# jdm365/Compression_Algorithms

Hardware: AMD Instinct MI355X
Metric: encode GB/s on enwik9 at 1/2/4/8 MI355X; ratio vs ref; round-trip bit-exact (higher is better)
Workload: dtype u8; 1 GPU; deflate (LZ77 W=32 KiB len<=31 + per-block dynamic Huffman over the 286-symbol alphabet, mode H), independent 64 KiB blocks; 1000000000 enwik-shaped bytes in the job, 1000000000 on rank 0; input_seed=12345, mode=H, input_bytes_job=1000000000, input_bytes_rank0=1000000000, compressed_bytes_job=516875560, compressed_bytes_rank0=516875560, gather_to_rank0=False, parallelism=blocks sharded over 1 GPU(s), weak scaling

## Files before the change

compression_algorithms_amd/csrc/lz2.h:

```cpp
#pragma once
#include "lz_common.h"

#define LZ2_NG_BITS   14
#define LZ2_NG        (1u << LZ2_NG_BITS)
#ifndef LZ2_CAP
#define LZ2_CAP       4096u
#endif
#ifndef LZ2_CAP_S
#define LZ2_CAP_S     2048u
#endif
#ifndef LZ2_THREADS
#define LZ2_THREADS   512
#endif
#define LZ2_NWAVES    (LZ2_THREADS / 64)
#ifndef LZ2_PARTBITS
#define LZ2_PARTBITS  7
#endif
#define LZ2_MAXPARTS  (1u << LZ2_PARTBITS)
static_assert(LZ2_CAP % LZ2_THREADS == 0 && LZ2_CAP_S % LZ2_THREADS == 0 && LZ2_CAP_S <= LZ2_CAP, "entries per thread must be whole");
static_assert(2u * (LZ_MAX_BLOCK / LZ2_CAP_S + 1u + 16u) + 2u <= LZ2_MAXPARTS, "a block could need more parts than the partition can number");
#define LZ2_GRID_PARTS 40u
static_assert(LZ2_GRID_PARTS * LZ2_CAP_S >= 5u * LZ_MAX_BLOCK / 4u, "the grid must cover a full block of text with room to spare");
#ifndef LZ2_BIG
#define LZ2_BIG       8u
#endif
#define LZ2_WAVE      128u
#define LZ2_MAXBIG    (LZ2_CAP / LZ2_BIG)
#define LZ2_BIG_STRIDE (2u * LZ_MAX_BLOCK)
#define LZ2_ALIGN8(x)  (((x) + 7u) & ~7u)
#define LZ2_DESC_SMALL (LZ_MAX_BLOCK / LZ2_BIG + 32u)
#define LZ2_NCLASS    8u
#define LZ2_BIG_SMALL 1024u
__host__ __device__ __forceinline__ uint32_t lz2_class_of(uint32_t cnt, uint32_t wave_min)
{
    const bool three = (wave_min >> 16) != 0u;
    wave_min &= 0xFFFFu;
    if (cnt >= wave_min) return cnt > LZ2_BIG_SMALL ? 6u : cnt >= 512u ? 4u : (three && cnt < 256u) ? 3u : 5u;
    return cnt < 16 ? 7u : cnt < 32 ? 0u : cnt < 64 ? 1u : cnt < 128 ? 2u : cnt < 256 ? 3u : 4u;
}

struct Lz2BlockMeta {
    uint32_t n, nparts, base, fallback;
    uint32_t nbig, nbig_entries;
    uint32_t pad[2];
    uint32_t part_start[LZ2_MAXPARTS];
    uint32_t part_count[LZ2_MAXPARTS];
    uint32_t part_lo[LZ2_MAXPARTS];
};

struct Lz2BigDesc {
    uint32_t block;
    uint32_t start;
    uint32_t count;
    uint32_t anom;
    uint32_t limit;
    uint32_t pad[3];
};

struct Lz2Scratch {
    uint8_t      *partmap;
    uint16_t     *plist;
    uint16_t     *cand;
    Lz2BlockMeta *meta;
    uint32_t     *fallback_count, *fallback_list;
    uint32_t     *work_count;
    uint32_t      work_slots;
    uint64_t     *work;
    uint16_t     *bigpos, *bigrs, *bigpid, *bigcand;
    Lz2BigDesc   *desc[LZ2_NCLASS];
    uint32_t     *big_count;
    uint64_t     *dbg;
    uint32_t      wave_min;
    uint32_t      stop_phase;
};
```

compression_algorithms_amd/csrc/lz2_find.hip:

```cpp
#include "lz_common.h"
#include "lz2.h"
#include "lz_dom.h"
#include "lz_replay.h"
#include <stdlib.h>

#define RS_HEAD 0x8000u
#define RS_MASK 0x7FFFu

__device__ __forceinline__ bool bm2_test(const uint32_t *bm, uint32_t b) { return (bm[b >> 5] >> (b & 31u)) & 1u; }

__device__ void replay_small(const uint16_t *pos, uint16_t *rs, const uint16_t *pid, uint16_t *occ, uint32_t *bm,
                             uint32_t s, uint32_t e, uint32_t W, uint32_t anom, uint32_t limit, uint16_t *cand_i)
{
    uint32_t ev = s;
    bool anom_pending = anom != ~0u;
    const bool plain = (anom == ~0u) && (limit == ~0u);
    if (plain && (uint32_t)pos[e - 1] <= (uint32_t)pos[s] + W) {
        for (uint32_t i = s; i < e; ++i) { const uint32_t id = pid[i]; cand_i[i] = (id != pos[i]) ? (uint16_t)id : (uint16_t)LZ_NONE16; }
        return;
    }
    for (uint32_t i = s; i < e; ++i) {
        const uint32_t p = pos[i], rsv = rs[i], r = rsv & RS_MASK, id = pid[i];
        while (ev < i && (uint32_t)pos[ev] + W < p) {
            const uint32_t b = rs[ev] & RS_MASK;
// ... 581 lines not shown
        lz2_find_part<LZ2_CAP>(in, n_total, P, sc, block0, k < nwide ? sc.work[sc.work_slots - 1u - k] : sc.work[covered + (k - nwide)]);
        __syncthreads();
    }
}

template <int LDS_ENTRIES, int NW>
__global__ __launch_bounds__(64)
void k_lz2_big(LzP P, Lz2Scratch sc, int large)
{
    __shared__ uint32_t s_occ[LDS_ENTRIES];
    __shared__ uint16_t s_slot[LDS_ENTRIES];
    const uint32_t lane = threadIdx.x;
    const uint32_t nhi = large == 1 ? sc.big_count[6] : (large == 2 || large == 4) ? 0u : sc.big_count[4],
                   ncl = nhi + ((large == 0 || large == 2) ? sc.big_count[5] : large == 4 ? sc.big_count[3] : 0u);
    const uint32_t W = 1u << P.wbits;
    for (uint32_t ci = blockIdx.x; ci < ncl; ci += gridDim.x) {
        const Lz2BigDesc *dp = large == 1 ? &sc.desc[6][ci] : large == 4 ? &sc.desc[3][ci] : (ci < nhi ? &sc.desc[4][ci] : &sc.desc[5][ci - nhi]);
        const uint32_t d_block = dp->block, d_start = dp->start, n = dp->count;
        if (n & 0x80000000u) continue;
        const uint32_t d_anom = dp->anom, d_limit = dp->limit;
        const uint16_t *bp = sc.bigpos + (size_t)d_block * LZ2_BIG_STRIDE + d_start;
        const uint16_t *br = sc.bigrs + (size_t)d_block * LZ2_BIG_STRIDE + d_start;
        const uint16_t *bi = sc.bigpid + (size_t)d_block * LZ2_BIG_STRIDE + d_start;
        uint16_t *bc = sc.bigcand + (size_t)d_block * LZ2_BIG_STRIDE + d_start;
        const bool plain = d_anom == ~0u && d_limit == ~0u;
        if constexpr (NW > 1) {
            if (n <= 2048u) {
                if (plain) big_replay<LDS_ENTRIES, 1, true>(s_occ, s_slot, lane, W, n, d_anom, d_limit, bp, br, bi, bc);
                else big_replay<LDS_ENTRIES, 1, false>(s_occ, s_slot, lane, W, n, d_anom, d_limit, bp, br, bi, bc);
                continue;
            }
            if (n <= 4096u) {
                if (plain) big_replay<LDS_ENTRIES, 2, true>(s_occ, s_slot, lane, W, n, d_anom, d_limit, bp, br, bi, bc);
                else big_replay<LDS_ENTRIES, 2, false>(s_occ, s_slot, lane, W, n, d_anom, d_limit, bp, br, bi, bc);
                continue;
            }
        }
        if (plain) big_replay<LDS_ENTRIES, NW, true>(s_occ, s_slot, lane, W, n, d_anom, d_limit, bp, br, bi, bc);
        else big_replay<LDS_ENTRIES, NW, false>(s_occ, s_slot, lane, W, n, d_anom, d_limit, bp, br, bi, bc);
    }
}

#define LZ2_DOM_DONE 0x80000000u
__global__ __launch_bounds__(256)
void k_lz2_dom(LzP P, Lz2Scratch sc)
{
    constexpr uint32_t RING = LZ2_CAP;
    static_assert((RING & (RING - 1u)) == 0, "the ring is indexed with a mask");
    __shared__ uint32_t s_occ[LZ2_CAP / 32 + 72 + 264];
    __shared__ uint16_t s_ring[RING];
    __shared__ uint16_t s_fid[DOM_FCAP], s_fpos[DOM_FCAP], s_fslot[DOM_FCAP];
    __shared__ uint32_t s_votes[3], s_result, s_next;
    const uint32_t tid = threadIdx.x;
    const uint32_t W = 1u << P.wbits;
    const uint32_t count = sc.big_count[6];
    uint32_t *cursor = sc.big_count + 8;
    struct Src {
        const uint16_t *bp, *br, *bi; uint16_t *bc;
        __device__ __forceinline__ uint64_t ent(uint32_t i) const { return ((uint64_t)bp[i] << 16) | ((uint64_t)br[i] << 32) | ((uint64_t)bi[i] << 48); }
        __device__ __forceinline__ void put(uint32_t i, uint32_t, uint32_t res) const { bc[i] = (uint16_t)res; }
    };
    for (;;) {
        __syncthreads();
        if (tid == 0) s_next = atomicAdd(cursor, 1u);
        __syncthreads();
        const uint32_t ci = s_next;
        if (ci >= count) break;
        Lz2BigDesc *dp = &sc.desc[6][ci];
        const uint32_t m = dp->count;
        if (dp->anom != ~0u || dp->limit != ~0u || m > LZ2_CAP) continue;
        const size_t at = (size_t)dp->block * LZ2_BIG_STRIDE + dp->start;
        Src src{sc.bigpos + at, sc.bigrs + at, sc.bigpid + at, sc.bigcand + at};
        for (uint32_t i = tid; i < m; i += 256) src.bc[i] = (uint16_t)LZ_NONE16;
        if (tid == 0) { s_votes[0] = s_votes[1] = s_votes[2] = 0; s_result = 0; }
        __syncthreads();
        const bool done = dom_cluster(src, m, W, (W < RING ? W : RING) - 1u, s_occ, s_ring, s_fid, s_fpos, s_fslot, s_votes, s_result, nullptr);
        if (done && tid == 0) dp->count = m | LZ2_DOM_DONE;
    }
}

#define ROW_BPERM(src_lane, v) ((uint32_t)__builtin_amdgcn_ds_bpermute((int)((src_lane) << 2), (int)(v)))

template <int RL>
__device__ __forceinline__ uint32_t row_first_zero(uint32_t v, uint32_t from, uint32_t l, uint32_t rb)
{
    constexpr uint32_t RMASK = RL == 32 ? 0xFFFFFFFFu : ((1u << (RL & 31)) - 1u);
    const uint32_t rw = from >> 5, lowmask = (1u << (from & 31u)) - 1u;
    if (l < rw) v = 0xFFFFFFFFu; else if (l == rw) v |= lowmask;
    const uint64_t mk = __ballot(v != 0xFFFFFFFFu);
    const uint32_t my = (uint32_t)(mk >> rb) & RMASK;
    const uint32_t ln = my ? (uint32_t)__builtin_ctz(my) : 0u;
    const uint32_t mv = ROW_BPERM(rb + ln, v);
    const uint32_t fz = (mv != 0xFFFFFFFFu) ? (uint32_t)__builtin_ctz(~mv) : 0u;
    return my ? ((ln << 5) + fz) : ~0u;
}

template <int RL>
__global__ __launch_bounds__(64)
void k_lz2_rows(LzP P, Lz2Scratch sc, int cls_a, int cls_b, int cursor_slot)
{
    static_assert(RL == 8 || RL == 16 || RL == 32, "rows of 8, 16 or 32 lanes");
    constexpr int NR = 64 / RL, CAPE = 32 * RL;
    constexpr uint32_t RMASK = RL == 32 ? 0xFFFFFFFFu : ((1u << (RL & 31)) - 1u);
    __shared__ uint32_t s_occ[NR][CAPE];
    __shared__ uint32_t s_ent[NR][CAPE];
    __shared__ uint32_t s_bm[NR][RL];
    const uint32_t lane = threadIdx.x, g = lane / (uint32_t)RL, l = lane & (uint32_t)(RL - 1), rb = lane & ~(uint32_t)(RL - 1);
    const uint32_t W = 1u << P.wbits;
    const uint32_t count_a = sc.big_count[cls_a], count = count_a + sc.big_count[cls_b];
    uint32_t *cursor = sc.big_count + cursor_slot;
    Lz2BigDesc *const descs_a = sc.desc[cls_a], *const descs_b = sc.desc[cls_b];
    auto desc_of = [&](uint32_t ticket) -> Lz2BigDesc * { return ticket < count_a ? descs_a + ticket : descs_b + (ticket - count_a); };
    uint32_t *occ = s_occ[g], *ent = s_ent[g], *bmw = s_bm[g];

    bool active = false, exhausted = false;
    uint32_t n = 0, i0 = 0, ev = 0;
    size_t at = 0;
    uint32_t cur_a = 0, cur_b = 0, out_acc = LZ_NONE16;
    uint32_t pf_stage = 0, pf_ci = 0, pf_count = 0;
    size_t pf_at = 0;
    uint32_t r_np = 0, r_ni = 0, r_nr = 0, r_fp = 0, r_fi = 0, r_fr = 0, tk = 0;
    uint4 r_d4 = make_uint4(0, 0, 0, 0); uint32_t r_d1 = 0;
    uint32_t vzero;
    asm volatile("v_mov_b32 %0, 0" : "=v"(vzero));

    for (;;) {
        const bool flush = active && i0 + l < n;
        uint16_t *const flush_to = sc.bigcand + at + i0 + l;
        if (active) {
            i0 += (uint32_t)RL;
            if (i0 >= n) active = false;
            else { cur_a = r_np | (r_ni << 16); cur_b = r_nr; }
        }
        bool take = false, want_cursor = false;
        uint32_t done_ci = 0, done_n = 0;
        if (!active && pf_stage == 3u) {
            take = true;
            n = pf_count; at = pf_at;
            cur_a = r_fp | (r_fi << 16); cur_b = r_fr; i0 = 0; ev = 0; active = true; pf_stage = 0;
            bmw[l] = 0;
            done_ci = pf_ci; done_n = n;
        }
        if (pf_stage == 1u) {
            pf_ci = ROW_BPERM(rb, tk);
            if (pf_ci >= count) { exhausted = true; pf_stage = 0; } else pf_stage = 2;
        } else if (pf_stage == 2u) {
            if (r_d4.w != ~0u || r_d1 != ~0u || r_d4.z > (uint32_t)CAPE || r_d4.z < 2u * RL) pf_stage = 0;
            else { pf_count = r_d4.z; pf_at = (size_t)r_d4.x * LZ2_BIG_STRIDE + r_d4.y; pf_stage = 3; }
        }
        if (pf_stage == 0u && !exhausted) { want_cursor = true; pf_stage = 1; }
        {
            const uint32_t k = i0 + (uint32_t)RL + l;
            const size_t na = (active && k < n) ? at + k : 0;
            r_np = sc.bigpos[na]; r_ni = sc.bigpid[na]; r_nr = sc.bigrs[na];
            const size_t fa = (pf_stage == 3u) ? pf_at + l : 0;
            r_fp = sc.bigpos[fa]; r_fi = sc.bigpid[fa]; r_fr = sc.bigrs[fa];
            const uint32_t *dp = reinterpret_cast<const uint32_t *>(pf_stage == 2u ? desc_of(pf_ci) : descs_a);
            r_d4 = *reinterpret_cast<const uint4 *>(dp); r_d1 = dp[4];
        }
        if (flush) *flush_to = (uint16_t)out_acc;
        if (take && l == 0) desc_of(done_ci)->count = done_n | LZ2_DOM_DONE;
        if (want_cursor && l == 0) tk = atomicAdd(cursor + vzero, 1u);
        if (__ballot(active || pf_stage != 0u) == 0ull) break;
        if (__ballot(active) == 0ull) continue;
        uint32_t a = ROW_BPERM(rb, cur_a), r = ROW_BPERM(rb, cur_b);
        uint32_t e = ent[(active && ev + l < i0) ? ev + l : 0u];
        for (uint32_t t = 0; t < (uint32_t)RL; ++t) {
            const uint32_t i = i0 + t;
            const bool on = active && i < n;
            const uint32_t p = a & 0xFFFFu, id = a >> 16;
            for (;;) {
                const bool ret = on && ev + l < i && (e >> 16) + W < p;
                const uint64_t mk = __ballot(ret);
                if (ret) atomicAnd(&bmw[(e & 0xFFFFu) >> 5], ~(1u << (e & 31u)));
                const uint32_t cnt = (uint32_t)__popc((uint32_t)(mk >> rb) & RMASK);
                ev += cnt;
                if (__ballot(cnt == (uint32_t)RL) == 0ull) break;
                e = ent[(on && ev + l < i) ? ev + l : 0u];
            }
            const uint32_t wr = bmw[r >> 5], h = occ[r], v = bmw[l];
            const uint32_t tn = (t + 1u) & (uint32_t)(RL - 1);
            const uint32_t na = ROW_BPERM(rb + tn, cur_a), nr = ROW_BPERM(rb + tn, cur_b);
            const bool bit = (wr >> (r & 31u)) & 1u, same = (h & 0xFFFFu) == id;
            const bool seek = on && id != p;
            uint32_t res = (seek && ev == 0u) ? id : (seek && bit && same) ? (h >> 16) : (uint32_t)LZ_NONE16;
            bool walk = seek && ev != 0u && bit && !same;
            if (__ballot(walk) != 0ull) {
                uint32_t e_end = row_first_zero<RL>(v, r + 1u, l, rb);
                if (e_end > (uint32_t)CAPE) e_end = (uint32_t)CAPE;
                uint32_t b0 = r + 1u;
                while (__ballot(walk && b0 < e_end) != 0ull) {
                    const uint32_t bb = b0 + l;
                    const bool in = walk && bb < e_end;
                    const uint32_t o = occ[in ? bb : 0u];
                    const uint64_t mk = __ballot(in && (o & 0xFFFFu) == id);
                    const uint32_t my = (uint32_t)(mk >> rb) & RMASK;
                    const uint32_t src = ROW_BPERM(rb + (my ? (uint32_t)__builtin_ctz(my) : 0u), o);
                    if (walk && my) { res = src >> 16; walk = false; }
                    b0 += (uint32_t)RL;
                }
            }
            const uint32_t b = row_first_zero<RL>(v, r, l, rb);
            const bool put = on && b < (uint32_t)CAPE;
            if (put && l == 0) atomicOr(&bmw[b >> 5], 1u << (b & 31u));
            if (put) { occ[b] = id | (p << 16); ent[i] = b | (p << 16); }
            if (on && l == t) out_acc = res;
            e = ent[(active && i + 1u < n && ev + l < i + 1u) ? ev + l : 0u];
            a = na; r = nr;
            __builtin_amdgcn_wave_barrier();
        }
    }
}

template <bool SMALL> struct SlotType { typedef uint8_t type; };
template <> struct SlotType<false> { typedef uint16_t type; };

__device__ __forceinline__ uint32_t u16_of(const uint4 &v, uint32_t k)
{
    const uint64_t lo = (uint64_t)v.x | ((uint64_t)v.y << 32), hi = (uint64_t)v.z | ((uint64_t)v.w << 32);
    return (uint32_t)(((k & 4u) ? hi : lo) >> ((k & 3u) * 16u)) & 0xFFFFu;
}

template <int CMAX, int LANES>
__global__ __launch_bounds__(64)
void k_lz2_mid_direct(LzP P, Lz2Scratch sc, int cls)
{
    constexpr int STRIDE = CMAX + 1;
    typedef typename SlotType<(CMAX <= 128)>::type slot_t;
    __shared__ uint32_t s_occ[LANES * STRIDE];
    __shared__ slot_t   s_slot[LANES * STRIDE];
    __shared__ uint32_t s_bits[LANES * (CMAX / 32 + 1)];
    const uint32_t lane = threadIdx.x;
    const uint32_t ncl = sc.big_count[cls];
    for (uint32_t wg = blockIdx.x; wg * (uint32_t)LANES < ncl; wg += gridDim.x) {
    const uint32_t ci = wg * (uint32_t)LANES + lane;
    const bool active = ci < ncl && lane < (uint32_t)LANES;
    struct { uint32_t block, start, count, anom, limit; } d = {0u, 0u, 0u, ~0u, ~0u};
    if (active) { const Lz2BigDesc *dp = &sc.desc[cls][ci]; d.block = dp->block; d.start = dp->start; d.count = dp->count; d.anom = dp->anom; d.limit = dp->limit; }
    const uint32_t n = d.count, W = 1u << P.wbits;
    const uint4 *vp = reinterpret_cast<const uint4 *>(sc.bigpos + (size_t)d.block * LZ2_BIG_STRIDE + d.start);
    const uint4 *vr = reinterpret_cast<const uint4 *>(sc.bigrs + (size_t)d.block * LZ2_BIG_STRIDE + d.start);
    const uint4 *vi = reinterpret_cast<const uint4 *>(sc.bigpid + (size_t)d.block * LZ2_BIG_STRIDE + d.start);
    uint4 *vc = reinterpret_cast<uint4 *>(sc.bigcand + (size_t)d.block * LZ2_BIG_STRIDE + d.start);
    const uint32_t lr = lane < (uint32_t)LANES ? lane : 0u;
    uint32_t *occ = s_occ + lr * STRIDE;
    slot_t *slot = s_slot + lr * STRIDE;
    uint32_t *bits = s_bits + lr * (CMAX / 32 + 1);
    if (lane < (uint32_t)LANES) for (int k = 0; k < CMAX / 32 + 1; ++k) bits[k] = 0;
    const uint4 zero4 = make_uint4(0, 0, 0, 0);
    uint4 evw = zero4;
    if (n) evw = vp[0];
    uint32_t ev = 0, ev_p = evw.x & 0xFFFFu;
    bool anom_pending = d.anom != ~0u;
    const bool plain = d.anom == ~0u && d.limit == ~0u;
    uint4 np = evw, nr = zero4, ni = zero4;
    if (n) { nr = vr[0]; ni = vi[0]; }
    for (uint32_t i0 = 0; i0 < (uint32_t)CMAX; i0 += 8) {
        if (__ballot(i0 < n) == 0ull) break;
        const uint4 cp = np, cr = nr, cid = ni;
        if (i0 + 8 < n) { np = vp[(i0 >> 3) + 1]; nr = vr[(i0 >> 3) + 1]; ni = vi[(i0 >> 3) + 1]; }
        uint32_t o0 = 0, o1 = 0, o2 = 0, o3 = 0;
#pragma unroll
        for (uint32_t k = 0; k < 8; ++k) {
            const uint32_t i = i0 + k;
            if (i < n) {
                const uint32_t p = u16_of(cp, k), r = u16_of(cr, k), id = u16_of(cid, k);
                while (ev < i && ev_p + W < p) {
                    const uint32_t b = slot[ev];
                    bits[b >> 5] &= ~(1u << (b & 31u));
                    ++ev;
                    if ((ev & 7u) == 0) evw = vp[ev >> 3];
                    ev_p = u16_of(evw, ev & 7u);
                }
                if (anom_pending && p > W - 1u) { bits[d.anom >> 5] &= ~(1u << (d.anom & 31u)); anom_pending = false; }
                uint32_t wi = r >> 5;
                const uint32_t w0 = bits[wi];
                uint32_t res = LZ_NONE16;
                if (plain && ev == 0) {
                    if (id != p) res = id;
                } else if (id != p && ((w0 >> (r & 31u)) & 1u)) {
                    for (uint32_t b = r;; ++b) {
                        if (b != r) {
                            if (b == d.limit && r < d.limit) break;
                            if (!((bits[b >> 5] >> (b & 31u)) & 1u)) break;
                        }
                        const uint32_t o = occ[b];
                        if ((o & 0xFFFFu) == id) { res = o >> 16; break; }
                    }
                }
                { const uint32_t v = res << ((k & 1u) * 16u); if (k < 2) o0 |= v; else if (k < 4) o1 |= v; else if (k < 6) o2 |= v; else o3 |= v; }
                uint32_t wv = w0 | ((1u << (r & 31u)) - 1u);
                while (wv == 0xFFFFFFFFu) wv = bits[++wi];
                const uint32_t b = (wi << 5) + (uint32_t)__builtin_ctz(~wv);
                bits[b >> 5] |= 1u << (b & 31u);
                occ[b] = id | (p << 16); slot[i] = (slot_t)b;
            }
        }
        if (i0 < n) vc[i0 >> 3] = make_uint4(o0, o1, o2, o3);
    }
    __builtin_amdgcn_wave_barrier();
    }
}

__global__ __launch_bounds__(1024)
void k_lz2_scatter(Lz2Scratch sc, uint16_t *__restrict__ cand_by_pos )
{
    const uint32_t lb = blockIdx.x;
    const Lz2BlockMeta *mt = sc.meta + lb;
    if (mt->fallback) return;
    const uint32_t n = mt->n;
    const uint16_t *pl = sc.plist + (size_t)lb * LZ_MAX_BLOCK, *cd = sc.cand + (size_t)lb * LZ_MAX_BLOCK;
    uint16_t *out = cand_by_pos + (size_t)lb * LZ_MAX_BLOCK;
    for (uint32_t j = threadIdx.x; j < n; j += 1024) { const uint32_t c = cd[j], p = pl[j]; if (c != p || p == LZ_NONE16) out[p] = (uint16_t)c; }
    __syncthreads();
    const uint32_t nb = mt->nbig_entries;
    const uint16_t *bp = sc.bigpos + (size_t)lb * LZ2_BIG_STRIDE, *bc = sc.bigcand + (size_t)lb * LZ2_BIG_STRIDE;
    for (uint32_t j = threadIdx.x; j < nb; j += 1024) { const uint32_t p = bp[j], c = bc[j]; if (c != p) out[p] = (uint16_t)c; }
}

template __global__ void k_lz2_mid_direct<16, 64>(LzP, Lz2Scratch, int);
template __global__ void k_lz2_mid_direct<32, 64>(LzP, Lz2Scratch, int);
template __global__ void k_lz2_mid_direct<64, 64>(LzP, Lz2Scratch, int);
template __global__ void k_lz2_mid_direct<128, 48>(LzP, Lz2Scratch, int);
template __global__ void k_lz2_big<LZ2_BIG_SMALL, 1>(LzP, Lz2Scratch, int);
template __global__ void k_lz2_big<512, 1>(LzP, Lz2Scratch, int);
template __global__ void k_lz2_big<256, 1>(LzP, Lz2Scratch, int);
template __global__ void k_lz2_big<LZ2_CAP, 4>(LzP, Lz2Scratch, int);
template __global__ void k_lz2_rows<16>(LzP, Lz2Scratch, int, int, int);


static uint32_t lz2_class_cap(uint32_t c)
{
    static const uint32_t lo[LZ2_NCLASS] = {16, 32, 64, 128, 256, 128, 1025, 8};
    return LZ_MAX_BLOCK / lo[c] + 8;
}

size_t lz2_scratch_bytes(uint32_t nb)
{
    size_t descs = 0;
    for (uint32_t c = 0; c < LZ2_NCLASS; ++c) descs += lz2_class_cap(c);
    return (size_t)nb * (LZ_MAX_BLOCK * (2 * 2 + 1) + LZ2_BIG_STRIDE * 2 * 4 + sizeof(Lz2BlockMeta) + 4 + 8 * LZ2_MAXPARTS + descs * sizeof(Lz2BigDesc)) + 16 * 256 + 4096 + 64 * 256;
}

void lz2_carve(mi_carver &cv, uint32_t nb, Lz2Scratch *sc)
{
    sc->partmap = cv.take<uint8_t>((size_t)nb * LZ_MAX_BLOCK);
    sc->plist = cv.take<uint16_t>((size_t)nb * LZ_MAX_BLOCK);
    sc->cand = cv.take<uint16_t>((size_t)nb * LZ_MAX_BLOCK);
    sc->meta = cv.take<Lz2BlockMeta>(nb);
    sc->fallback_count = cv.take<uint32_t>(64);
    sc->fallback_list = cv.take<uint32_t>(nb);
    sc->bigpos = cv.take<uint16_t>((size_t)nb * LZ2_BIG_STRIDE);
    sc->bigrs = cv.take<uint16_t>((size_t)nb * LZ2_BIG_STRIDE);
    sc->bigpid = cv.take<uint16_t>((size_t)nb * LZ2_BIG_STRIDE);
    sc->bigcand = cv.take<uint16_t>((size_t)nb * LZ2_BIG_STRIDE);
    for (uint32_t c = 0; c < LZ2_NCLASS; ++c) sc->desc[c] = cv.take<Lz2BigDesc>((size_t)nb * lz2_class_cap(c));
    sc->big_count = sc->fallback_count + 16;
    sc->work_count = sc->fallback_count + 32;
    sc->work = cv.take<uint64_t>((size_t)nb * LZ2_MAXPARTS);
    sc->work_slots = nb * LZ2_MAXPARTS;
    sc->dbg = getenv("MI_LZ_DEBUG") ? cv.take<uint64_t>(64) : nullptr;
    { const char *e = getenv("MI_LZ_ROWS"); const uint32_t rows = e ? (uint32_t)atoi(e) : 1u; sc->wave_min = LZ2_WAVE | ((rows ? 1u : 0u) << 16); }
#ifdef MI_MEASURE
    sc->stop_phase = getenv("MI_LZ_STOP_PHASE") ? (uint32_t)atoi(getenv("MI_LZ_STOP_PHASE")) : 0u;
#else
    sc->stop_phase = 0u;
#endif
}

static uint32_t lz2_env_u32(const char *name, uint32_t dflt)
{
    const char *e = getenv(name);
    if (!e) return dflt;
    const long v = atol(e);
    return v >= 0 ? (uint32_t)v : dflt;
}

extern "C" int mi_lz_debug_counters(mi_ctx *ctx, uint64_t *out32)
{
    if (!ctx || !ctx->lz_dbg) return 0;
    (void)hipDeviceSynchronize();
    return hipMemcpy(out32, ctx->lz_dbg, 64 * 8, hipMemcpyDeviceToHost) == hipSuccess ? 1 : 0;
}

void lz2_launch_partition(const uint8_t *d_in, uint64_t n, const LzP &P, const Lz2Scratch &sc, uint64_t block0, uint32_t nb, hipStream_t s);

mi_status lz2_stage_partition(mi_ctx *ctx, const LzP &P, const uint8_t *d_in, uint64_t n, uint64_t block0, uint32_t nb,
                              const Lz2Scratch &sc, hipStream_t s)
{
    MI_HIP(ctx, hipMemsetAsync(sc.fallback_count, 0, 256, s));
    if (sc.dbg && ctx->lz_dbg != sc.dbg) { ctx->lz_dbg = sc.dbg; MI_HIP(ctx, hipMemsetAsync(sc.dbg, 0, 512, s)); }
    mi_prof_scope p(ctx, "k_lz2_partition", s, (uint64_t)nb * P.block);
    lz2_launch_partition(d_in, n, P, sc, block0, nb, s);
    MI_HIP(ctx, hipGetLastError());
    return MI_OK;
}

static uint32_t lz2_find_grid(const LzP &P, uint32_t nb)
{
    const uint32_t parts = P.block / 64u + 1u < LZ2_GRID_PARTS ? P.block / 64u + 1u : LZ2_GRID_PARTS;
    return (parts * nb + 7u) & ~7u;
}

mi_status lz2_stage_find(mi_ctx *ctx, const LzP &P, const uint8_t *d_in, uint64_t n, uint64_t block0, uint32_t nb,
                         const Lz2Scratch &sc, hipStream_t s)
{
    mi_prof_scope p(ctx, "k_lz2_find", s, (uint64_t)nb * P.block);
    hipLaunchKernelGGL(k_lz2_find, dim3(lz2_find_grid(P, nb)), dim3(LZ2_THREADS), 0, s, d_in, n, P, sc, block0);
    MI_HIP(ctx, hipGetLastError());
    return MI_OK;
}

mi_status lz2_stage_find_wide(mi_ctx *ctx, const LzP &P, const uint8_t *d_in, uint64_t n, uint64_t block0, uint32_t nb,
                              const Lz2Scratch &sc, hipStream_t s, bool aside)
{
    static const bool prof_fb = getenv("MI_LZ_PROF_FALLBACK") != nullptr;
    const int saved_prof = ctx->profiling;
    if (aside && !prof_fb) ctx->profiling = 0;
    {
        mi_prof_scope p(ctx, "k_lz2_find_wide", s, (uint64_t)nb * P.block);
        hipLaunchKernelGGL(k_lz2_find_wide, dim3(256), dim3(LZ2_THREADS), 0, s, d_in, n, P, sc, block0, lz2_find_grid(P, nb));
    }
    ctx->profiling = saved_prof;
    MI_HIP(ctx, hipGetLastError());
    return MI_OK;
}

mi_status lz2_stage_b(mi_ctx *ctx, const LzP &P, uint32_t nb, const Lz2Scratch &sc, hipStream_t s, int which)
{
    const uint32_t ncu = (uint32_t)ctx->num_cu;
    auto grid_of = [&](uint64_t worst) -> uint32_t {
        const uint64_t g = (uint64_t)ncu * lz2_env_u32("MI_LZ_REPLAY_WAVES", 0);
        return (uint32_t)((g == 0 || worst < g) ? (worst ? worst : 1) : g);
    };
    if (which & 1) {
    { mi_prof_scope p(ctx, "k_lz2_mid<16>", s, (uint64_t)nb * P.block);
      hipLaunchKernelGGL((k_lz2_mid_direct<16, 64>), dim3(grid_of((uint64_t)nb * lz2_class_cap(7) / 64 + 1)), dim3(64), 0, s, P, sc, 7); }
    { mi_prof_scope p(ctx, "k_lz2_mid<32>", s, (uint64_t)nb * P.block);
      hipLaunchKernelGGL((k_lz2_mid_direct<32, 64>), dim3(grid_of((uint64_t)nb * lz2_class_cap(0) / 64 + 1)), dim3(64), 0, s, P, sc, 0); }
    }
    if (which & 4) {
    { mi_prof_scope p(ctx, "k_lz2_mid<64>", s, (uint64_t)nb * P.block);
      hipLaunchKernelGGL((k_lz2_mid_direct<64, 64>), dim3(grid_of((uint64_t)nb * lz2_class_cap(1) / 64 + 1)), dim3(64), 0, s, P, sc, 1); }
    { mi_prof_scope p(ctx, "k_lz2_mid<128>", s, (uint64_t)nb * P.block);
      hipLaunchKernelGGL((k_lz2_mid_direct<128, 48>), dim3(grid_of((uint64_t)nb * lz2_class_cap(2) / 48 + 1)), dim3(64), 0, s, P, sc, 2); }
    }
    if (which & 2) {
    { mi_prof_scope p(ctx, "k_lz2_big", s, (uint64_t)nb * P.block);
      static const bool split = !(getenv("MI_LZ_BIG_SPLIT") && getenv("MI_LZ_BIG_SPLIT")[0] == '0');
      const uint32_t rows = sc.wave_min >> 16;
      static const uint32_t rows_waves = lz2_env_u32("MI_LZ_ROWS_WAVES", 9);
      if (rows >= 1 && split && (sc.wave_min & 0xFFFFu) == LZ2_WAVE) {
          hipLaunchKernelGGL((k_lz2_big<LZ2_BIG_SMALL, 1>), dim3(grid_of((uint64_t)nb * lz2_class_cap(4))), dim3(64), 0, s, P, sc, 3);
          hipLaunchKernelGGL((k_lz2_rows<16>), dim3(ncu * rows_waves), dim3(64), 0, s, P, sc, 5, 3, 9);
          hipLaunchKernelGGL((k_lz2_big<512, 1>), dim3(ncu * 4u), dim3(64), 0, s, P, sc, 2);
          hipLaunchKernelGGL((k_lz2_big<256, 1>), dim3(ncu * 4u), dim3(64), 0, s, P, sc, 4);
      } else if (split && (sc.wave_min & 0xFFFFu) == LZ2_WAVE) {
          hipLaunchKernelGGL((k_lz2_big<LZ2_BIG_SMALL, 1>), dim3(grid_of((uint64_t)nb * lz2_class_cap(4))), dim3(64), 0, s, P, sc, 3);
          hipLaunchKernelGGL((k_lz2_big<512, 1>), dim3(grid_of((uint64_t)nb * lz2_class_cap(5))), dim3(64), 0, s, P, sc, 2);
      } else {
          hipLaunchKernelGGL((k_lz2_big<LZ2_BIG_SMALL, 1>), dim3(grid_of((uint64_t)nb * (lz2_class_cap(4) + lz2_class_cap(5)))), dim3(64), 0, s, P, sc, 0);
          if (rows) hipLaunchKernelGGL((k_lz2_big<256, 1>), dim3(grid_of((uint64_t)nb * lz2_class_cap(3))), dim3(64), 0, s, P, sc, 4);
      } }
    { mi_prof_scope p(ctx, "k_lz2_dom", s, (uint64_t)nb * P.block);
      const uint64_t worst = (uint64_t)nb * lz2_class_cap(6);
      hipLaunchKernelGGL(k_lz2_dom, dim3((unsigned)(worst < (uint64_t)ncu * 4u ? worst : (uint64_t)ncu * 4u)), dim3(256), 0, s, P, sc); }
    { mi_prof_scope p(ctx, "k_lz2_big<4096>", s, (uint64_t)nb * P.block);
      hipLaunchKernelGGL((k_lz2_big<LZ2_CAP, 4>), dim3(grid_of((uint64_t)nb * lz2_class_cap(6) < 4096 ? (uint64_t)nb * lz2_class_cap(6) : 4096)), dim3(64), 0, s, P, sc, 1); }
    }
    MI_HIP(ctx, hipGetLastError());
    return MI_OK;
}

void lz2_launch_scatter(const Lz2Scratch &sc, uint16_t *cand_by_pos, uint32_t nb, hipStream_t s)
{
    hipLaunchKernelGGL(k_lz2_scatter, dim3(nb), dim3(1024), 0, s, sc, cand_by_pos);
}
```

Baseline: 23.11 GB/s.

## Replace per-class mid replay kernels with exact-size lane-sorted replay

```diff
diff --git a/compression_algorithms_amd/csrc/lz2.h b/compression_algorithms_amd/csrc/lz2.h
--- a/compression_algorithms_amd/csrc/lz2.h
+++ b/compression_algorithms_amd/csrc/lz2.h
@@ -69,6 +69,8 @@
     uint16_t     *bigpos, *bigrs, *bigpid, *bigcand;
     Lz2BigDesc   *desc[LZ2_NCLASS];
     uint32_t     *big_count;
+    uint4        *lane_list;
+    uint32_t     *lane_hist;
     uint64_t     *dbg;
     uint32_t      wave_min;
     uint32_t      stop_phase;
diff --git a/compression_algorithms_amd/csrc/lz2_find.hip b/compression_algorithms_amd/csrc/lz2_find.hip
--- a/compression_algorithms_amd/csrc/lz2_find.hip
+++ b/compression_algorithms_amd/csrc/lz2_find.hip
@@ -907,6 +907,159 @@
     }
 }
 
+constexpr uint32_t LANE_SIZES = LZ2_WAVE;
+
+__host__ __device__ __forceinline__ uint32_t lz2_lane_region(uint32_t n)
+{
+    return ((n + 1u) + ((n + 32u) >> 5) + ((n + 3u) >> 2)) | 1u;
+}
+__host__ __device__ __forceinline__ uint32_t lz2_lane_width(uint32_t n, uint32_t budget_dw)
+{
+    const uint32_t l = budget_dw / lz2_lane_region(n);
+    return l < 64u ? l : 64u;
+}
+
+__device__ __forceinline__ const Lz2BigDesc *lz2_lane_desc(const Lz2Scratch &sc, uint32_t v, uint32_t n7, uint32_t n0, uint32_t n1)
+{
+    if (v < n7) return sc.desc[7] + v;
+    v -= n7;
+    if (v < n0) return sc.desc[0] + v;
+    v -= n0;
+    if (v < n1) return sc.desc[1] + v;
+    return sc.desc[2] + (v - n1);
+}
+
+__global__ __launch_bounds__(256)
+void k_lz2_lane_count(Lz2Scratch sc)
+{
+    __shared__ uint32_t s_h[LANE_SIZES];
+    const uint32_t tid = threadIdx.x;
+    const uint32_t n7 = sc.big_count[7], n0 = sc.big_count[0], n1 = sc.big_count[1], N = n7 + n0 + n1 + sc.big_count[2];
+    if (blockIdx.x * 256u >= N) return;
+    if (tid < LANE_SIZES) s_h[tid] = 0;
+    __syncthreads();
+    for (uint32_t v = blockIdx.x * 256u + tid; v < N; v += gridDim.x * 256u)
+        atomicAdd(&s_h[lz2_lane_desc(sc, v, n7, n0, n1)->count & (LANE_SIZES - 1u)], 1u);
+    __syncthreads();
+    if (tid < LANE_SIZES && s_h[tid]) atomicAdd(&sc.lane_hist[tid], s_h[tid]);
+}
+
+__global__ __launch_bounds__(256)
+void k_lz2_lane_place(LzP P, Lz2Scratch sc)
+{
+    __shared__ uint32_t s_h[LANE_SIZES], s_at[LANE_SIZES];
+    const uint32_t tid = threadIdx.x;
+    const uint32_t n7 = sc.big_count[7], n0 = sc.big_count[0], n1 = sc.big_count[1], N = n7 + n0 + n1 + sc.big_count[2];
+    if (blockIdx.x * 256u >= N) return;
+    if (tid < LANE_SIZES) s_h[tid] = 0;
+    __syncthreads();
+    for (uint32_t v = blockIdx.x * 256u + tid; v < N; v += gridDim.x * 256u)
+        atomicAdd(&s_h[lz2_lane_desc(sc, v, n7, n0, n1)->count & (LANE_SIZES - 1u)], 1u);
+    __syncthreads();
+    if (tid < 64u) {
+        const uint32_t a = LANE_SIZES - 1u - 2u * tid, b = a - 1u;
+        const uint32_t ha = sc.lane_hist[a], hb = sc.lane_hist[b];
+        const uint32_t before = wave_inclusive_scan<uint32_t>(ha + hb, OpAddU32(), 0u) - ha - hb;
+        if (s_h[a]) s_at[a] = before + atomicAdd(&sc.lane_hist[LANE_SIZES + a], s_h[a]);
+        if (s_h[b]) s_at[b] = before + ha + atomicAdd(&sc.lane_hist[LANE_SIZES + b], s_h[b]);
+        s_h[a] = 0; s_h[b] = 0;
+    }
+    __syncthreads();
+    for (uint32_t v = blockIdx.x * 256u + tid; v < N; v += gridDim.x * 256u) {
+        const Lz2BigDesc *dp = lz2_lane_desc(sc, v, n7, n0, n1);
+        const uint32_t c = dp->count & (LANE_SIZES - 1u), at = s_at[c] + atomicAdd(&s_h[c], 1u);
+        if (at >= N) { lz_order_violation(P); continue; }
+        sc.lane_list[at] = make_uint4(dp->block, dp->start, dp->count, (dp->anom & 0xFFFFu) | (dp->limit << 16));
+    }
+}
+
+__global__ __launch_bounds__(64)
+void k_lz2_lanes(LzP P, Lz2Scratch sc, uint32_t size_hi, uint32_t size_lo, uint32_t budget_dw)
+{
+    extern __shared__ uint32_t s_lane[];
+    const uint32_t lane = threadIdx.x;
+    const uint32_t a = LANE_SIZES - 1u - 2u * lane, b = a - 1u;
+    const uint32_t ha = sc.lane_hist[a], hb = sc.lane_hist[b];
+    const uint32_t wa = (a <= size_hi && a >= size_lo) ? (ha + lz2_lane_width(a, budget_dw) - 1u) / lz2_lane_width(a, budget_dw) : 0u;
+    const uint32_t wb = (b <= size_hi && b >= size_lo) ? (hb + lz2_lane_width(b, budget_dw) - 1u) / lz2_lane_width(b, budget_dw) : 0u;
+    const uint32_t hin = wave_inclusive_scan<uint32_t>(ha + hb, OpAddU32(), 0u);
+    const uint32_t win = wave_inclusive_scan<uint32_t>(wa + wb, OpAddU32(), 0u);
+    const uint32_t g = blockIdx.x;
+    if (g >= (uint32_t)__builtin_amdgcn_readlane((int)win, 63)) return;
+    const uint32_t j = (uint32_t)__popcll(__ballot(win <= g));
+    const uint32_t wj = (uint32_t)__builtin_amdgcn_readlane((int)win, (int)j), waj = (uint32_t)__builtin_amdgcn_readlane((int)wa, (int)j),
+                   wbj = (uint32_t)__builtin_amdgcn_readlane((int)wb, (int)j), hj = (uint32_t)__builtin_amdgcn_readlane((int)hin, (int)j),
+                   haj = (uint32_t)__builtin_amdgcn_readlane((int)ha, (int)j), hbj = (uint32_t)__builtin_amdgcn_readlane((int)hb, (int)j);
+    const uint32_t q0 = g - (wj - waj - wbj);
+    const bool upper = q0 < waj;
+    const uint32_t n = LANE_SIZES - 1u - 2u * j - (upper ? 0u : 1u), q = upper ? q0 : q0 - waj, hn = upper ? haj : hbj;
+    const uint32_t first = (hj - haj - hbj) + (upper ? 0u : haj);
+    const uint32_t width = lz2_lane_width(n, budget_dw), k0 = q * width, nl = (hn - k0 < width) ? hn - k0 : width;
+    uint4 dv = make_uint4(0u, 0u, 0u, 0xFFFFFFFFu);
+    if (lane < nl) dv = sc.lane_list[first + k0 + lane];
+    if (lane < nl && dv.z != n) lz_order_violation(P);
+    const uint32_t cnt = (lane < nl && dv.z == n) ? n : 0u, W = 1u << P.wbits;
+    const uint32_t anom = (dv.w & 0xFFFFu) == 0xFFFFu ? ~0u : (dv.w & 0xFFFFu), limit = (dv.w >> 16) == 0xFFFFu ? ~0u : (dv.w >> 16);
+    const uint4 *vp = reinterpret_cast<const uint4 *>(sc.bigpos + (size_t)dv.x * LZ2_BIG_STRIDE + dv.y);
+    const uint4 *vr = reinterpret_cast<const uint4 *>(sc.bigrs + (size_t)dv.x * LZ2_BIG_STRIDE + dv.y);
+    const uint4 *vi = reinterpret_cast<const uint4 *>(sc.bigpid + (size_t)dv.x * LZ2_BIG_STRIDE + dv.y);
+    uint4 *vc = reinterpret_cast<uint4 *>(sc.bigcand + (size_t)dv.x * LZ2_BIG_STRIDE + dv.y);
+    uint32_t *occ = s_lane + (cnt ? lane : 0u) * lz2_lane_region(n);
+    uint32_t *bits = occ + (n + 1u);
+    uint8_t *slot = reinterpret_cast<uint8_t *>(bits + ((n + 32u) >> 5));
+    if (cnt) for (uint32_t k = 0; k < ((n + 32u) >> 5); ++k) bits[k] = 0;
+    const uint4 zero4 = make_uint4(0, 0, 0, 0);
+    uint4 evw = zero4;
+    if (cnt) evw = vp[0];
+    uint32_t ev = 0, ev_p = evw.x & 0xFFFFu;
+    bool anom_pending = anom != ~0u;
+    const bool plain = anom == ~0u && limit == ~0u;
+    uint4 np = evw, nr = zero4, ni = zero4;
+    if (cnt) { nr = vr[0]; ni = vi[0]; }
+    for (uint32_t i0 = 0; i0 < n; i0 += 8) {
+        const uint4 cp = np, cr = nr, cid = ni;
+        if (i0 + 8 < cnt) { np = vp[(i0 >> 3) + 1]; nr = vr[(i0 >> 3) + 1]; ni = vi[(i0 >> 3) + 1]; }
+        uint32_t o0 = 0, o1 = 0, o2 = 0, o3 = 0;
+#pragma unroll
+        for (uint32_t k = 0; k < 8; ++k) {
+            const uint32_t i = i0 + k;
+            if (i < cnt) {
+                const uint32_t p = u16_of(cp, k), r = u16_of(cr, k), id = u16_of(cid, k);
+                while (ev < i && ev_p + W < p) {
+                    const uint32_t sb = slot[ev];
+                    bits[sb >> 5] &= ~(1u << (sb & 31u));
+                    ++ev;
+                    if ((ev & 7u) == 0) evw = vp[ev >> 3];
+                    ev_p = u16_of(evw, ev & 7u);
+                }
+                if (anom_pending && p > W - 1u) { bits[anom >> 5] &= ~(1u << (anom & 31u)); anom_pending = false; }
+                uint32_t wi = r >> 5;
+                const uint32_t w0 = bits[wi];
+                uint32_t res = LZ_NONE16;
+                if (plain && ev == 0) {
+                    if (id != p) res = id;
+                } else if (id != p && ((w0 >> (r & 31u)) & 1u)) {
+                    for (uint32_t sb = r;; ++sb) {
+                        if (sb != r) {
+                            if (sb == limit && r < limit) break;
+                            if (!((bits[sb >> 5] >> (sb & 31u)) & 1u)) break;
+                        }
+                        const uint32_t o = occ[sb];
+                        if ((o & 0xFFFFu) == id) { res = o >> 16; break; }
+                    }
+                }
+                { const uint32_t v = res << ((k & 1u) * 16u); if (k < 2) o0 |= v; else if (k < 4) o1 |= v; else if (k < 6) o2 |= v; else o3 |= v; }
+                uint32_t wv = w0 | ((1u << (r & 31u)) - 1u);
+                while (wv == 0xFFFFFFFFu) wv = bits[++wi];
+                const uint32_t sb = (wi << 5) + (uint32_t)__builtin_ctz(~wv);
+                bits[sb >> 5] |= 1u << (sb & 31u);
+                occ[sb] = id | (p << 16); slot[i] = (uint8_t)sb;
+            }
+        }
+        if (i0 < cnt) vc[i0 >> 3] = make_uint4(o0, o1, o2, o3);
+    }
+}
+
 __global__ __launch_bounds__(1024)
 void k_lz2_scatter(Lz2Scratch sc, uint16_t *__restrict__ cand_by_pos )
 {
@@ -944,7 +1097,8 @@
 {
     size_t descs = 0;
     for (uint32_t c = 0; c < LZ2_NCLASS; ++c) descs += lz2_class_cap(c);
-    return (size_t)nb * (LZ_MAX_BLOCK * (2 * 2 + 1) + LZ2_BIG_STRIDE * 2 * 4 + sizeof(Lz2BlockMeta) + 4 + 8 * LZ2_MAXPARTS + descs * sizeof(Lz2BigDesc)) + 16 * 256 + 4096 + 64 * 256;
+    return (size_t)nb * (LZ_MAX_BLOCK * (2 * 2 + 1) + LZ2_BIG_STRIDE * 2 * 4 + sizeof(Lz2BlockMeta) + 4 + 8 * LZ2_MAXPARTS + descs * sizeof(Lz2BigDesc)
+                         + lz2_class_cap(7) * sizeof(uint4)) + 16 * 256 + 4096 + 64 * 256 + 2 * LANE_SIZES * 4 + 256;
 }
 
 void lz2_carve(mi_carver &cv, uint32_t nb, Lz2Scratch *sc)
@@ -953,7 +1107,7 @@
     sc->plist = cv.take<uint16_t>((size_t)nb * LZ_MAX_BLOCK);
     sc->cand = cv.take<uint16_t>((size_t)nb * LZ_MAX_BLOCK);
     sc->meta = cv.take<Lz2BlockMeta>(nb);
-    sc->fallback_count = cv.take<uint32_t>(64);
+    sc->fallback_count = cv.take<uint32_t>(64 + 2 * LANE_SIZES);
     sc->fallback_list = cv.take<uint32_t>(nb);
     sc->bigpos = cv.take<uint16_t>((size_t)nb * LZ2_BIG_STRIDE);
     sc->bigrs = cv.take<uint16_t>((size_t)nb * LZ2_BIG_STRIDE);
@@ -962,8 +1116,10 @@
     for (uint32_t c = 0; c < LZ2_NCLASS; ++c) sc->desc[c] = cv.take<Lz2BigDesc>((size_t)nb * lz2_class_cap(c));
     sc->big_count = sc->fallback_count + 16;
     sc->work_count = sc->fallback_count + 32;
+    sc->lane_hist = sc->fallback_count + 64;
     sc->work = cv.take<uint64_t>((size_t)nb * LZ2_MAXPARTS);
     sc->work_slots = nb * LZ2_MAXPARTS;
+    sc->lane_list = cv.take<uint4>((size_t)nb * lz2_class_cap(7));
     sc->dbg = getenv("MI_LZ_DEBUG") ? cv.take<uint64_t>(64) : nullptr;
     { const char *e = getenv("MI_LZ_ROWS"); const uint32_t rows = e ? (uint32_t)atoi(e) : 1u; sc->wave_min = LZ2_WAVE | ((rows ? 1u : 0u) << 16); }
 #ifdef MI_MEASURE
@@ -993,7 +1149,7 @@
 mi_status lz2_stage_partition(mi_ctx *ctx, const LzP &P, const uint8_t *d_in, uint64_t n, uint64_t block0, uint32_t nb,
                               const Lz2Scratch &sc, hipStream_t s)
 {
-    MI_HIP(ctx, hipMemsetAsync(sc.fallback_count, 0, 256, s));
+    MI_HIP(ctx, hipMemsetAsync(sc.fallback_count, 0, (64 + 2 * LANE_SIZES) * 4, s));
     if (sc.dbg && ctx->lz_dbg != sc.dbg) { ctx->lz_dbg = sc.dbg; MI_HIP(ctx, hipMemsetAsync(sc.dbg, 0, 512, s)); }
     mi_prof_scope p(ctx, "k_lz2_partition", s, (uint64_t)nb * P.block);
     lz2_launch_partition(d_in, n, P, sc, block0, nb, s);
@@ -1038,13 +1194,28 @@
         const uint64_t g = (uint64_t)ncu * lz2_env_u32("MI_LZ_REPLAY_WAVES", 0);
         return (uint32_t)((g == 0 || worst < g) ? (worst ? worst : 1) : g);
     };
-    if (which & 1) {
+    static const bool lanes = !(getenv("MI_LZ_LANES") && getenv("MI_LZ_LANES")[0] == '0');
+    if (lanes && (which & 4)) {
+        static const uint32_t kib_env = lz2_env_u32("MI_LZ_LANES_KIB", 8);
+        const uint32_t kib = kib_env < 1u ? 1u : kib_env > 32u ? 32u : kib_env, budget_dw = kib * 256u;
+        const uint64_t worst = (uint64_t)nb * lz2_class_cap(7);
+        const uint32_t og = (uint32_t)((worst + 255u) / 256u < (uint64_t)ncu * 4u ? (worst + 255u) / 256u : (uint64_t)ncu * 4u);
+        { mi_prof_scope p(ctx, "k_lz2_lane_order", s, (uint64_t)nb * P.block);
+          hipLaunchKernelGGL(k_lz2_lane_count, dim3(og), dim3(256), 0, s, sc);
+          hipLaunchKernelGGL(k_lz2_lane_place, dim3(og), dim3(256), 0, s, P, sc); }
+        uint32_t m = ~0u;
+        for (uint32_t c = LZ2_BIG; c < LANE_SIZES; ++c) { const uint32_t x = c * lz2_lane_width(c, budget_dw); m = x < m ? x : m; }
+        const uint64_t waves = (uint64_t)nb * LZ_MAX_BLOCK / m + LANE_SIZES;
+        { mi_prof_scope p(ctx, "k_lz2_lanes", s, (uint64_t)nb * P.block);
+          hipLaunchKernelGGL(k_lz2_lanes, dim3((uint32_t)waves), dim3(64), budget_dw * 4u, s, P, sc, LANE_SIZES - 1u, LZ2_BIG, budget_dw); }
+    }
+    if (!lanes && (which & 1)) {
     { mi_prof_scope p(ctx, "k_lz2_mid<16>", s, (uint64_t)nb * P.block);
       hipLaunchKernelGGL((k_lz2_mid_direct<16, 64>), dim3(grid_of((uint64_t)nb * lz2_class_cap(7) / 64 + 1)), dim3(64), 0, s, P, sc, 7); }
     { mi_prof_scope p(ctx, "k_lz2_mid<32>", s, (uint64_t)nb * P.block);
       hipLaunchKernelGGL((k_lz2_mid_direct<32, 64>), dim3(grid_of((uint64_t)nb * lz2_class_cap(0) / 64 + 1)), dim3(64), 0, s, P, sc, 0); }
     }
-    if (which & 4) {
+    if (!lanes && (which & 4)) {
     { mi_prof_scope p(ctx, "k_lz2_mid<64>", s, (uint64_t)nb * P.block);
       hipLaunchKernelGGL((k_lz2_mid_direct<64, 64>), dim3(grid_of((uint64_t)nb * lz2_class_cap(1) / 64 + 1)), dim3(64), 0, s, P, sc, 1); }
     { mi_prof_scope p(ctx, "k_lz2_mid<128>", s, (uint64_t)nb * P.block);
```

Result: faster. 23.78 GB/s, median of 6 (+2.9%).
